# rvignolo/RayTracing.jl

Hardware: NVIDIA B200
Metric: segments/sec for segmentize! (higher is better)
Workload: dtype f64

## Files before the change

### raytracing.jl_b200/csrc/march.cuh

```cuda
#pragma once
#include "topo.cuh"

namespace rt {

#ifndef RT_MARCH_THREADS
#define RT_MARCH_THREADS 32
#endif
constexpr int kMarchThreads = RT_MARCH_THREADS;
#ifndef RT_MARCH_WAIT
#define RT_MARCH_WAIT 6
#endif
constexpr int kMarchWait = RT_MARCH_WAIT;
#ifndef RT_MARCH_MIN_BLOCKS
#define RT_MARCH_MIN_BLOCKS 32
#endif

struct MarchState {
    double ta, tb, tc, g, ang_thr;
    long long t, cidx;
    int j, az, limit, stop_cell;
    bool right, cheap_ok;
    double s1, s2;
    int enc, last_rec;
    float clearA;
    int f;
    int live;
    int active;
    double qx, qy;
    int cur, cur_kout;
    int mode, nseg, pb, endcode, status, n_litpush;
    int recording;
    unsigned lit_iters, nn_q, knn_q;
    unsigned s_rec;
};

enum { MODE_RETRY = 3 };

__device__ __forceinline__ void sts32(unsigned addr, int v) { asm volatile("st.shared.b32 [%0], %1;" ::"r"(addr), "r"(v) : "memory"); }
__device__ __forceinline__ int lds32(unsigned addr) {
    int v;
    asm volatile("ld.shared.b32 %0, [%1];" : "=r"(v) : "r"(addr) : "memory");
    return v;
}

__device__ __forceinline__ void march_push(const WalkParams &P, bool at_stop, int rec, int &nseg, int &pb, int &recording, int &mode,
                                           int &endcode, int limit, unsigned s_rec) {
    if (recording) {
        if (nseg > 0 && (nseg & (kRecBlock - 1)) == 0) {
            const int nb = atomicAdd(P.pool_cursor, 1);
            if (nb >= P.pool_blocks) {
                recording = 0;
            } else {
                P.pool_next[pb] = nb;
                pb = nb;
            }
        }
        if (recording) {
            const int k = nseg & 7;
            sts32(s_rec + 4u * kMarchThreads * k, rec);
            if (k == 7) {
                int v[8];
#pragma unroll
                for (int q = 0; q < 8; ++q) v[q] = lds32(s_rec + 4u * kMarchThreads * q);
                stg256_plain_i(P.pool + (long long)pb * kRecBlock + ((nseg & (kRecBlock - 1)) - 7), v);
            }
        }
    }
    nseg += 1;
    if (nseg >= limit) {
        endcode = END_CAP;
        mode = MODE_DONE;
    } else if (at_stop) {
        endcode = END_HANDOFF;
        mode = MODE_DONE;
    }
}

__device__ __forceinline__ void march_arm(const DevMesh &m, MarchState &s, int e, int e_q, bool &clean) {
    const CellRec &r = m.cells[e];
    s.cur = e;
    s.cur_kout = e_q;
    s.last_rec = -1;
    s.clearA = fabsf(r.clear);
    const double v0 = s.ta * r.vx[0] + s.tb * r.vy[0] + s.tc, v1 = s.ta * r.vx[1] + s.tb * r.vy[1] + s.tc,
                 v2 = s.ta * r.vx[2] + s.tb * r.vy[2] + s.tc;
    const double thr = s.g * (double)s.clearA;
    s.s1 = e_q == 0 ? v0 : (e_q == 1 ? v1 : v2);
    s.s2 = e_q == 0 ? v1 : (e_q == 1 ? v2 : v0);
    clean = (fabs(v0) >= thr) && (fabs(v1) >= thr) && (fabs(v2) >= thr) && ((s.s1 > 0) != (s.s2 > 0));
    s.enc = m.twin[3 * e + e_q];
    s.f = s.enc & 1;
}

__device__ __forceinline__ bool march_exact(const WalkParams &P, double ta, double tb, double tc, int h, bool exit1, bool right, float clearf) {
    const DevMesh &m = P.m;
    const int cellB = h / 3;
    const int kin = h - 3 * cellB;
    int kout = kin + (exit1 ? 1 : 2);
    kout = kout >= 3 ? kout - 3 : kout;
    const Line trk{ta, tb, tc};
    const EdgeRec ei = m.edges[3 * cellB + kin], eo = m.edges[3 * cellB + kout];
    P2 pi, X;
    const bool par_i = intersection(trk, Line{ei.a, ei.b, ei.c}, pi);
    const bool par_o = intersection(trk, Line{eo.a, eo.b, eo.c}, X);
    const bool kin_lt_kout = (kin == 0) || (kin == 1 && exit1);
    const bool in_first = right ? (kin_lt_kout ? (pi.x < X.x) : !(X.x < pi.x)) : (kin_lt_kout ? (pi.x > X.x) : !(X.x > pi.x));
    const double l = norm2(pi.x - X.x, pi.y - X.y);
    bool accept = !par_i && !par_o && in_first && l > P.lmin;
    if (accept && clearf < 0.0f) accept = bbox_dist(m, pi.x, pi.y) > 0.25 * l + 8.0 * P.tiny;
    return accept;
}

__device__ __noinline__ void march_slow(const WalkParams &P, MarchState &s) {
    const DevMesh &m = P.m;
    const unsigned long long pol_keep = l2_policy_keep();
    const bool literal_only = (P.flags & 1u) != 0;
    if (s.mode == MODE_RETRY && s.enc >= 0) {
        double ax, ay, w0, w1;
        ldg256_keep(m.he + (s.enc >> 3), pol_keep, ax, ay, w0, w1);
        const float clearf = __int_as_float(__double2loint(w1));
        const float clearB = fabsf(clearf);
        const double sa = s.ta * ax + s.tb * ay + s.tc;
        const double thr = s.g * (double)fmaxf(s.clearA, clearB);
        if ((fabs(sa) >= thr) && (fabs(s.s1) >= thr) && (fabs(s.s2) >= thr)) {
            const bool opp1 = (sa > 0) != (s.s1 > 0);
            const double ks = opp1 ? s.s1 : s.s2;
            const bool exit1 = (opp1 == (s.f != 0));
            const int nenc = exit1 ? __double2loint(w0) : __double2hiint(w0);
            const int h = s.enc >> 3;
            const int cellB = h / 3;
            const bool accept = march_exact(P, s.ta, s.tb, s.tc, h, exit1, s.right, clearf);
            if (accept) {
                s.s1 = ks;
                s.s2 = sa;
                s.f = (exit1 == ((nenc & 1) != 0)) ? 1 : 0;
                s.enc = nenc;
                s.clearA = clearB;
                s.last_rec = (h << 2) | (exit1 ? 2 : 0);
                s.mode = MODE_FAST;
                march_push(P, cellB == s.stop_cell, s.last_rec, s.nseg, s.pb, s.recording, s.mode, s.endcode, s.limit, s.s_rec);
                return;
            }
        }
    }
    s.mode = MODE_SLOW;
    if (s.last_rec >= 0) {
        const int r = s.last_rec;
        const int h = r >> 2;
        const int cell = h / 3;
        const int kin = h - 3 * cell;
        int kout = kin + ((r & 2) ? 1 : 2);
        kout = kout >= 3 ? kout - 3 : kout;
        const P2 X = exit_point(m, Line{s.ta, s.tb, s.tc}, cell, kout);
        s.cur = cell;
        s.cur_kout = kout;
        s.qx = X.x;
        s.qy = X.y;
        s.last_rec = -1;
    }
    LitIn in{s.ta, s.tb, s.tc, P.tiny * P.ang.cosp[s.az], P.tiny * P.ang.sinp[s.az], s.qx, s.qy, s.cur, s.right, s.j == 0 && s.nseg == 0};
    LitOut o;
    literal_until_push(P, in, o);
    s.lit_iters += o.iters;
    s.nn_q += (unsigned)o.nq[0];
    s.knn_q += (unsigned)o.nq[1];
    if (o.code == 0) {
        s.n_litpush++;
        march_push(P, o.e == s.stop_cell, (o.e << 2) | 1, s.nseg, s.pb, s.recording, s.mode, s.endcode, s.limit, s.s_rec);
        s.cur = o.e;
        s.cur_kout = o.e_q;
        s.qx = o.qx;
        s.qy = o.qy;
        s.last_rec = -1;
        if (s.mode != MODE_DONE && !literal_only && o.e_q >= 0) {
            bool clean;
            march_arm(m, s, o.e, o.e_q, clean);
            if (clean) s.mode = MODE_FAST;
        }
    } else {
        s.endcode = o.code;
        s.status = o.status;
        s.mode = MODE_DONE;
    }
}

__device__ __noinline__ void march_init(const WalkParams &P, MarchState &s, int lane, long long unit) {
    const DevMesh &m = P.m;
    const int blk = P.ch.unit_block[unit];
    s.j = (int)(unit - P.ch.unit_base[blk]);
    s.t = 32LL * blk + lane;
    s.cidx = unit * 32 + lane;
    s.mode = MODE_DONE;
    s.nseg = 0;
    s.status = 0;
    s.endcode = END_TRACK;
    s.n_litpush = 0;
    s.lit_iters = s.nn_q = s.knn_q = 0;
    s.enc = -1;
    s.last_rec = -1;
    s.cur = -1;
    s.cur_kout = -1;
    s.stop_cell = -1;
    s.limit = P.max_iter;
    s.pb = (int)(s.cidx - P.pool_slot_base);
    s.recording = 1;
    s.ta = s.tb = s.tc = s.g = s.ang_thr = s.s1 = s.s2 = s.qx = s.qy = 0.0;
    s.clearA = INFINITY;
    s.f = 0;
    s.right = true;
    s.cheap_ok = false;
    s.az = 0;
    s.live = s.active = 0;
    const long long t = s.t;
    if (t >= P.n_tracks) return;
    const int n = P.ch.nch[t];
    if (s.j >= n) return;
    s.live = 1;
    if (t < P.trk_begin || t >= P.trk_end) return;
    const int seed = s.j == 0 ? -2 : P.ch.seed_cell[s.cidx];
    if (seed == -1) return;
    s.active = 1;
    constexpr double kKappa = 1.0 / RT_KAPPA_INV;
    s.az = P.t.azim[t];
    s.ta = P.t.a[t];
    s.tb = P.t.b[t];
    s.tc = P.t.c[t];
    s.right = P.ang.phi[s.az] < kPi / 2;
    s.g = sqrt(s.ta * s.ta + s.tb * s.tb);
    s.ang_thr = kKappa * s.g * P.lmax;
    s.cheap_ok = P.lmin * (fabs(s.tb) / s.g) > 32.0 * 2.220446049250313e-16 * P.smax / kKappa;
    const bool literal_only = (P.flags & 1u) != 0;
    if (s.j == 0) {
        s.qx = P.t.px[t];
        s.qy = P.t.py[t];
        s.mode = MODE_SLOW;
    } else {
        bool clean;
        march_arm(m, s, seed, P.ch.seed_kexit[s.cidx], clean);
        s.qx = P.ch.seed_qx[s.cidx];
        s.qy = P.ch.seed_qy[s.cidx];
        s.mode = (literal_only || !clean) ? MODE_SLOW : MODE_FAST;
    }
    for (int jj = s.j + 1; jj < n; ++jj) {
        const int sc = P.ch.seed_cell[s.cidx + 32LL * (jj - s.j)];
        if (sc >= 0) {
            s.stop_cell = sc;
            break;
        }
    }
    if (s.j > 0 && s.stop_cell == s.cur) {
        s.endcode = END_HANDOFF;
        s.mode = MODE_DONE;
    }
    if (s.limit <= 0) {
        s.endcode = END_CAP;
        s.mode = MODE_DONE;
    }
}

__global__ void __launch_bounds__(kMarchThreads, RT_MARCH_MIN_BLOCKS) k_march(const __grid_constant__ WalkParams P) {
    const unsigned FULL = 0xffffffffu;
    const DevMesh &m = P.m;
    __shared__ int s_rec[8 * kMarchThreads];
    const int lane = threadIdx.x & 31;
    const long long gw = (blockIdx.x * (long long)blockDim.x + threadIdx.x) >> 5;
    const long long slot = P.unit_begin + gw;
    if (slot >= P.unit_end) return;
    const long long unit = P.ch.order ? P.ch.order[slot] : slot;

    MarchState S;
    S.s_rec = (unsigned)__cvta_generic_to_shared(s_rec + threadIdx.x);
    march_init(P, S, lane, unit);
    const bool live = S.live != 0, active = S.active != 0;

    double ta = S.ta, tb = S.tb, tc = S.tc, g = S.g, ang_thr = S.ang_thr;
    bool cheap_ok = S.cheap_ok;
    int limit = S.limit, stop_cell = S.stop_cell;
    unsigned my_rec = S.s_rec;
    double s1 = S.s1, s2 = S.s2;
    int enc = S.enc, last_rec = S.last_rec, mode = S.mode, nseg = S.nseg, pb = S.pb, endcode = S.endcode;
    float clearA = S.clearA;
    int f = S.f, recording = S.recording;
    const unsigned long long pol_keep = l2_policy_keep();
#ifdef RT_MARCH_DIAG
    unsigned diag_tot = 0, diag_done = 0, diag_wait = 0;
#endif

    double rax = 0.0, ray = 0.0, rw0 = 0.0, rw1 = 0.0;
    if (mode == MODE_FAST && enc >= 0) ldg256_keep(m.he + (enc >> 3), pol_keep, rax, ray, rw0, rw1);

    while (__any_sync(FULL, mode != MODE_DONE)) {
#pragma unroll 1
        for (int it = 0; it < 4 * kFastBatch; ++it) {
            if (!__any_sync(FULL, mode == MODE_FAST)) break;
            if ((it & 1) && __popc(__ballot_sync(FULL, mode == MODE_SLOW || mode == MODE_RETRY)) >= kMarchWait) break;
#ifdef RT_MARCH_DIAG
            diag_tot++;
            if (mode == MODE_DONE) diag_done++;
            else if (mode != MODE_FAST) diag_wait++;
#endif
            if (mode != MODE_FAST) continue;
            if (enc < 0) {
                mode = MODE_RETRY;
                continue;
            }
            const double sa = ta * rax + tb * ray + tc;
            const bool opp1 = (sa > 0) != (s1 > 0);
            const bool exit1 = (opp1 == (f != 0));
            const int nenc = exit1 ? __double2loint(rw0) : __double2hiint(rw0);
            const float clearf = __int_as_float(__double2loint(rw1));
            const float clear2 = __int_as_float(__double2hiint(rw1));
#ifndef RT_MARCH_LATE_LOAD
            if (nenc >= 0) ldg256_keep(m.he + (nenc >> 3), pol_keep, rax, ray, rw0, rw1);
#endif
            const float clearB = fabsf(clearf);
            const double thr = g * (double)fmaxf(clearA, clearB);
            const double ks = opp1 ? s1 : s2;
#ifdef RT_MARCH_BRANCHY
            const bool accept = (fabs(sa) >= thr) && (fabs(s1) >= thr) && (fabs(s2) >= thr) && cheap_ok && (clearf >= 0.0f) &&
                                (fabs(ks) >= g * (double)clear2) && (fabs(ks) + fabs(sa) >= ang_thr) && (fabs(s1) + fabs(s2) >= ang_thr);
#else
            const bool accept = (fabs(sa) >= thr) & (fabs(s1) >= thr) & (fabs(s2) >= thr) & cheap_ok & (clearf >= 0.0f) &
                                (fabs(ks) >= g * (double)clear2) & (fabs(ks) + fabs(sa) >= ang_thr) & (fabs(s1) + fabs(s2) >= ang_thr);
#endif
            if (!accept) {
                mode = MODE_RETRY;
                continue;
            }
            const int h = enc >> 3;
            last_rec = (h << 2) | (exit1 ? 2 : 0);
            s1 = ks;
            s2 = sa;
            f = (exit1 == ((nenc & 1) != 0)) ? 1 : 0;
            enc = nenc;
            clearA = clearB;
            const bool at_stop = (unsigned)(h - 3 * stop_cell) < 3u;
            march_push(P, at_stop, last_rec, nseg, pb, recording, mode, endcode, limit, my_rec);
#ifdef RT_MARCH_LATE_LOAD
            if (mode == MODE_FAST && enc >= 0) ldg256_keep(m.he + (enc >> 3), pol_keep, rax, ray, rw0, rw1);
#endif
        }
        if (mode == MODE_SLOW || mode == MODE_RETRY) {
            S.s1 = s1;
            S.s2 = s2;
            S.enc = enc;
            S.last_rec = last_rec;
            S.clearA = clearA;
            S.f = f;
            S.mode = mode;
            S.nseg = nseg;
            S.pb = pb;
            S.recording = recording;
            S.endcode = endcode;
            march_slow(P, S);
            ta = S.ta;
            tb = S.tb;
            tc = S.tc;
            g = S.g;
            ang_thr = S.ang_thr;
            cheap_ok = S.cheap_ok;
            limit = S.limit;
            stop_cell = S.stop_cell;
            my_rec = S.s_rec;
            s1 = S.s1;
            s2 = S.s2;
            enc = S.enc;
            last_rec = S.last_rec;
            clearA = S.clearA;
            f = S.f;
            mode = S.mode;
            nseg = S.nseg;
            pb = S.pb;
            recording = S.recording;
            endcode = S.endcode;
            rax = ray = rw0 = rw1 = 0.0;
            if (mode == MODE_FAST && enc >= 0) ldg256_keep(m.he + (enc >> 3), pol_keep, rax, ray, rw0, rw1);
        }
    }

    if (recording && (nseg & 7)) {
        const int rem = nseg & 7;
        int *dst = P.pool + (long long)pb * kRecBlock + (((nseg - 1) & (kRecBlock - 1)) - (rem - 1));
        for (int kk = 0; kk < rem; ++kk) dst[kk] = lds32(my_rec + 4u * kMarchThreads * kk);
    }
    if (live) {
        P.ch.count[S.cidx] = active ? nseg : 0;
        P.ch.sum[S.cidx] = 0.0;
        P.ch.endcode[S.cidx] = active ? (endcode | (S.status << 8)) : (END_HANDOFF | (0 << 8));
    } else {
        P.ch.count[S.cidx] = 0;
    }
    if (P.counters) {
        unsigned long long v = active ? (unsigned long long)(nseg - S.n_litpush) : 0ull;
        unsigned long long li = S.lit_iters, q0 = S.nn_q, q1 = S.knn_q;
#ifdef RT_MARCH_DIAG
        li = diag_done;
        q0 = diag_wait;
        q1 = diag_tot;
#endif
        for (int o = 16; o > 0; o >>= 1) {
            v += __shfl_down_sync(FULL, v, o);
            li += __shfl_down_sync(FULL, li, o);
            q0 += __shfl_down_sync(FULL, q0, o);
            q1 += __shfl_down_sync(FULL, q1, o);
        }
        if (lane == 0) {
            if (v) atomicAdd(&P.counters[0], v);
            if (li) atomicAdd(&P.counters[1], li);
            if (q0) atomicAdd(&P.counters[2], q0);
            if (q1) atomicAdd(&P.counters[3], q1);
        }
    }
}

}
```

Before: 33.15 billion.

## Use conservatively rounded float thresholds and merged warp votes in fast march loop

Moves the fast-path acceptance tests from double to float. Thresholds are rounded up and magnitudes rounded down, so the test stays conservative, and cheap_ok is folded into an infinite angle threshold. It also caches |s1| and |s2| as floats, checks the stop cell against the encoded half-edge directly, and replaces two per-iteration warp votes with a single ballot whose break condition counts lanes no longer in fast mode. The aim is to cut FP64 work and warp-synchronisation overhead in the hot loop. In exchange, a few more crossings may fall back to the slow path because the float bounds are looser, and the loop-exit policy changes.

```diff
diff --git a/raytracing.jl_b200/csrc/march.cuh b/raytracing.jl_b200/csrc/march.cuh
--- a/raytracing.jl_b200/csrc/march.cuh
+++ b/raytracing.jl_b200/csrc/march.cuh
@@ -16,10 +16,11 @@
 #endif
 
 struct MarchState {
-    double ta, tb, tc, g, ang_thr;
+    double ta, tb, tc, g;
+    float gf, angf;
     long long t, cidx;
     int j, az, limit, stop_cell;
-    bool right, cheap_ok;
+    bool right;
     double s1, s2;
     int enc, last_rec;
     float clearA;
@@ -204,11 +205,11 @@
     s.limit = P.max_iter;
     s.pb = (int)(s.cidx - P.pool_slot_base);
     s.recording = 1;
-    s.ta = s.tb = s.tc = s.g = s.ang_thr = s.s1 = s.s2 = s.qx = s.qy = 0.0;
+    s.ta = s.tb = s.tc = s.g = s.s1 = s.s2 = s.qx = s.qy = 0.0;
+    s.gf = s.angf = INFINITY;
     s.clearA = INFINITY;
     s.f = 0;
     s.right = true;
-    s.cheap_ok = false;
     s.az = 0;
     s.live = s.active = 0;
     const long long t = s.t;
@@ -227,8 +228,10 @@
     s.tc = P.t.c[t];
     s.right = P.ang.phi[s.az] < kPi / 2;
     s.g = sqrt(s.ta * s.ta + s.tb * s.tb);
-    s.ang_thr = kKappa * s.g * P.lmax;
-    s.cheap_ok = P.lmin * (fabs(s.tb) / s.g) > 32.0 * 2.220446049250313e-16 * P.smax / kKappa;
+    s.gf = nextafterf(__double2float_ru(s.g), INFINITY);
+    const double ang_thr = kKappa * s.g * P.lmax;
+    const bool cheap_ok = P.lmin * (fabs(s.tb) / s.g) > 32.0 * 2.220446049250313e-16 * P.smax / kKappa;
+    s.angf = cheap_ok ? __double2float_ru(ang_thr) : INFINITY;
     const bool literal_only = (P.flags & 1u) != 0;
     if (s.j == 0) {
         s.qx = P.t.px[t];
@@ -273,72 +276,85 @@
     march_init(P, S, lane, unit);
     const bool live = S.live != 0, active = S.active != 0;
 
-    double ta = S.ta, tb = S.tb, tc = S.tc, g = S.g, ang_thr = S.ang_thr;
-    bool cheap_ok = S.cheap_ok;
-    int limit = S.limit, stop_cell = S.stop_cell;
-    unsigned my_rec = S.s_rec;
-    double s1 = S.s1, s2 = S.s2;
-    int enc = S.enc, last_rec = S.last_rec, mode = S.mode, nseg = S.nseg, pb = S.pb, endcode = S.endcode;
-    float clearA = S.clearA;
-    int f = S.f, recording = S.recording;
+    double ta, tb, tc, s1, s2;
+    float gf, angf, clearA, a1, a2;
+    int stop24, limit, enc, last_rec, mode, nseg, pb, endcode, f, recording;
+    unsigned my_rec;
     const unsigned long long pol_keep = l2_policy_keep();
 #ifdef RT_MARCH_DIAG
     unsigned diag_tot = 0, diag_done = 0, diag_wait = 0;
 #endif
 
-    double rax = 0.0, ray = 0.0, rw0 = 0.0, rw1 = 0.0;
-    if (mode == MODE_FAST && enc >= 0) ldg256_keep(m.he + (enc >> 3), pol_keep, rax, ray, rw0, rw1);
-
-    while (__any_sync(FULL, mode != MODE_DONE)) {
+    double rax, ray, rw0, rw1;
+    auto load_hot = [&]() {
+        ta = S.ta;
+        tb = S.tb;
+        tc = S.tc;
+        gf = S.gf;
+        angf = S.angf;
+        limit = S.limit;
+        stop24 = 24 * S.stop_cell;
+        my_rec = S.s_rec;
+        s1 = S.s1;
+        s2 = S.s2;
+        enc = S.enc;
+        last_rec = S.last_rec;
+        clearA = S.clearA;
+        f = S.f;
+        mode = S.mode;
+        nseg = S.nseg;
+        pb = S.pb;
+        recording = S.recording;
+        endcode = S.endcode;
+        a1 = __double2float_rd(fabs(s1));
+        a2 = __double2float_rd(fabs(s2));
+        if (mode == MODE_FAST && (enc < 0 || !(__fadd_rd(a1, a2) >= angf))) mode = MODE_RETRY;
+        rax = ray = rw0 = rw1 = 0.0;
+        if (mode == MODE_FAST) ldg256_keep(m.he + (enc >> 3), pol_keep, rax, ray, rw0, rw1);
+    };
+    load_hot();
+
+    for (;;) {
+        const unsigned not_done = __ballot_sync(FULL, mode != MODE_DONE);
+        if (!not_done) break;
+        const int wait_max = min(kMarchWait, __popc(not_done));
 #pragma unroll 1
         for (int it = 0; it < 4 * kFastBatch; ++it) {
-            if (!__any_sync(FULL, mode == MODE_FAST)) break;
-            if ((it & 1) && __popc(__ballot_sync(FULL, mode == MODE_SLOW || mode == MODE_RETRY)) >= kMarchWait) break;
 #ifdef RT_MARCH_DIAG
             diag_tot++;
             if (mode == MODE_DONE) diag_done++;
             else if (mode != MODE_FAST) diag_wait++;
 #endif
-            if (mode != MODE_FAST) continue;
-            if (enc < 0) {
-                mode = MODE_RETRY;
-                continue;
+            if (mode == MODE_FAST) {
+                const float clearf = __int_as_float(__double2loint(rw1));
+                const float clearB = fabsf(clearf);
+                const float thr = __fmul_ru(gf, fmaxf(clearA, clearB));
+                const float thr2 = __fmul_ru(gf, __int_as_float(__double2hiint(rw1)));
+                const double sa = ta * rax + tb * ray + tc;
+                const bool opp1 = (sa > 0) != (s1 > 0);
+                const bool exit1 = (opp1 == (f != 0));
+                const int nenc = exit1 ? __double2loint(rw0) : __double2hiint(rw0);
+                if (nenc >= 0) ldg256_keep(m.he + (nenc >> 3), pol_keep, rax, ray, rw0, rw1);
+                const float asa = __double2float_rd(fabs(sa));
+                const float aks = opp1 ? a1 : a2;
+                const bool accept = (enc >= 0) & (asa >= thr) & (fminf(a1, a2) >= thr) & (clearf >= 0.0f) & (aks >= thr2) &
+                                    (__fadd_rd(aks, asa) >= angf);
+                if (!accept) {
+                    mode = MODE_RETRY;
+                } else {
+                    const bool at_stop = (unsigned)(enc - stop24) < 24u;
+                    last_rec = ((enc >> 3) << 2) | (exit1 ? 2 : 0);
+                    s1 = opp1 ? s1 : s2;
+                    s2 = sa;
+                    a1 = aks;
+                    a2 = asa;
+                    f = (exit1 == ((nenc & 1) != 0)) ? 1 : 0;
+                    enc = nenc;
+                    clearA = clearB;
+                    march_push(P, at_stop, last_rec, nseg, pb, recording, mode, endcode, limit, my_rec);
+                }
             }
-            const double sa = ta * rax + tb * ray + tc;
-            const bool opp1 = (sa > 0) != (s1 > 0);
-            const bool exit1 = (opp1 == (f != 0));
-            const int nenc = exit1 ? __double2loint(rw0) : __double2hiint(rw0);
-            const float clearf = __int_as_float(__double2loint(rw1));
-            const float clear2 = __int_as_float(__double2hiint(rw1));
-#ifndef RT_MARCH_LATE_LOAD
-            if (nenc >= 0) ldg256_keep(m.he + (nenc >> 3), pol_keep, rax, ray, rw0, rw1);
-#endif
-            const float clearB = fabsf(clearf);
-            const double thr = g * (double)fmaxf(clearA, clearB);
-            const double ks = opp1 ? s1 : s2;
-#ifdef RT_MARCH_BRANCHY
-            const bool accept = (fabs(sa) >= thr) && (fabs(s1) >= thr) && (fabs(s2) >= thr) && cheap_ok && (clearf >= 0.0f) &&
-                                (fabs(ks) >= g * (double)clear2) && (fabs(ks) + fabs(sa) >= ang_thr) && (fabs(s1) + fabs(s2) >= ang_thr);
-#else
-            const bool accept = (fabs(sa) >= thr) & (fabs(s1) >= thr) & (fabs(s2) >= thr) & cheap_ok & (clearf >= 0.0f) &
-                                (fabs(ks) >= g * (double)clear2) & (fabs(ks) + fabs(sa) >= ang_thr) & (fabs(s1) + fabs(s2) >= ang_thr);
-#endif
-            if (!accept) {
-                mode = MODE_RETRY;
-                continue;
-            }
-            const int h = enc >> 3;
-            last_rec = (h << 2) | (exit1 ? 2 : 0);
-            s1 = ks;
-            s2 = sa;
-            f = (exit1 == ((nenc & 1) != 0)) ? 1 : 0;
-            enc = nenc;
-            clearA = clearB;
-            const bool at_stop = (unsigned)(h - 3 * stop_cell) < 3u;
-            march_push(P, at_stop, last_rec, nseg, pb, recording, mode, endcode, limit, my_rec);
-#ifdef RT_MARCH_LATE_LOAD
-            if (mode == MODE_FAST && enc >= 0) ldg256_keep(m.he + (enc >> 3), pol_keep, rax, ray, rw0, rw1);
-#endif
+            if (__popc(not_done & ~__ballot_sync(FULL, mode == MODE_FAST)) >= wait_max) break;
         }
         if (mode == MODE_SLOW || mode == MODE_RETRY) {
             S.s1 = s1;
@@ -353,28 +369,7 @@
             S.recording = recording;
             S.endcode = endcode;
             march_slow(P, S);
-            ta = S.ta;
-            tb = S.tb;
-            tc = S.tc;
-            g = S.g;
-            ang_thr = S.ang_thr;
-            cheap_ok = S.cheap_ok;
-            limit = S.limit;
-            stop_cell = S.stop_cell;
-            my_rec = S.s_rec;
-            s1 = S.s1;
-            s2 = S.s2;
-            enc = S.enc;
-            last_rec = S.last_rec;
-            clearA = S.clearA;
-            f = S.f;
-            mode = S.mode;
-            nseg = S.nseg;
-            pb = S.pb;
-            recording = S.recording;
-            endcode = S.endcode;
-            rax = ray = rw0 = rw1 = 0.0;
-            if (mode == MODE_FAST && enc >= 0) ldg256_keep(m.he + (enc >> 3), pol_keep, rax, ray, rw0, rw1);
+            load_hot();
         }
     }
 
```

Result: faster. 33.78 billion, median of 6 (+1.9%).
